# WinnerBy/PreGANPlus

Hardware: AMD Instinct MI355X
Metric: host-windows/sec (detect+diagnose+generate) (higher is better)
Workload: dtype fp32; 1 GPU; C2: PreGAN+ batched inference, 50 hosts x W=3 x 3 resources, 65536 windows per GPU, fp32; windows_per_gpu=65536, parallelism=dp1 (independent windows)

## Files before the change

preganplus_amd/csrc/pgp_decoder.hip:

```cpp
#include "pgp_device.hpp"

namespace pgp {
namespace {

constexpr int kDecWaves = 16;

template <int H>
constexpr int dec_cps() {
  int best = 1;
  for (int c = 1; c * Geo<H>::DEC_G <= 16; ++c)
    if ((H * kWindow) % c == 0) best = c;
  return best;
}

template <int H>
struct DecLds {
  static constexpr int CPS = dec_cps<H>();
  static constexpr int SLOT = CPS * Geo<H>::DEC_G * Geo<H>::FQ;
  static constexpr int TAB = Geo<H>::t_size(kMaxProtos);
  static constexpr int TOTAL = 2 * SLOT + TAB;
};

template <int H>
__global__ __launch_bounds__(kDecWaves * 64, H <= 16 ? 8 : 1) void decoder_kernel(FwdArgs a) {
  using G = Geo<H>;
  using L = DecLds<H>;
  __shared__ __attribute__((aligned(16))) float smem[L::TOTAL];
  float* tab = smem + 2 * L::SLOT;
  const int tsz = G::t_size(a.K);
  for (int i = threadIdx.x; i < tsz; i += blockDim.x) tab[i] = a.tab[i];

  const int lane = threadIdx.x & 63, g = lane >> 4, j = lane & 15;
  const int wv = __builtin_amdgcn_readfirstlane(threadIdx.x >> 6);
  const long blk = (long)blockIdx.x * kDecWaves + wv;
  const long nblk = (a.B + 15) / 16;
  const bool active = blk < nblk;
  const float* wdec = a.frags + G::OFF_DEC;
  const float* lat = a.lat + (active ? blk : 0) * G::LAT_BLK;
  constexpr int NCH = H * kWindow;

  constexpr int CPS = L::CPS, SG = CPS * G::DEC_G;
  float* cur = smem;
  float* nxt = smem + L::SLOT;
  dma_groups(wdec, cur, SG, wv, kDecWaves, lane);
  auto load_b = [&](int c, bool ok, float (&v)[G::KS_D]) {
    const float* lc = lat + (long)c * G::KS_D * 64;
#pragma unroll
    for (int q = 0; q < G::LAT_FG; ++q) {
      const f32x4 t = ok ? ld4(lc + q * 256 + lane * 4) : f32x4{0.f, 0.f, 0.f, 0.f};
#pragma unroll
      for (int e = 0; e < 4; ++e) v[4 * q + e] = t[e];
    }
#pragma unroll
    for (int r = 0; r < G::KS_D % 4; ++r) v[4 * G::LAT_FG + r] = ok ? lc[G::LAT_FG * 256 + r * 64 + lane] : 0.f;
  };
  float b[CPS][G::KS_D];
#pragma unroll
  for (int u = 0; u < CPS; ++u) load_b(u, active, b[u]);
  __syncthreads();
  if (CPS < NCH) dma_groups(wdec + (long)SG * G::FQ, nxt, SG, wv, kDecWaves, lane);

  f32x4 acc[G::MT_O];
#pragma unroll
  for (int mt = 0; mt < G::MT_O; ++mt) acc[mt] = f32x4{0.f, 0.f, 0.f, 0.f};
  constexpr int MTM = G::MT_O;

#pragma unroll 1
  for (int c0 = 0; c0 < NCH; c0 += CPS) {
    float bn[CPS][G::KS_D];
    const bool pre = active && (c0 + CPS < NCH);
#pragma unroll
    for (int u = 0; u < CPS; ++u) load_b(c0 + CPS + u, pre, bn[u]);
#pragma unroll
    for (int sub = 0; sub < CPS; ++sub) {
      const float* A = cur + sub * G::DEC_G * G::FQ;
      constexpr int AMAX = G::MT_O >= 16 ? 4 : H <= 16 ? 2 : 7;
      constexpr int NGRP = (MTM + AMAX - 1) / AMAX;
      constexpr int MH = (MTM + NGRP - 1) / NGRP;
#pragma unroll
      for (int q4 = 0; q4 < G::KQ_D; ++q4) {
#pragma unroll
        for (int m0 = 0; m0 < MTM; m0 += MH) {
          f32x4 av[MH];
#pragma unroll
          for (int i = 0; i < MH; ++i)
            if (m0 + i < MTM) av[i] = ld4(A + ((m0 + i) * G::KQ_D + q4) * 256 + lane * 4);
#pragma unroll
          for (int e = 0; e < 4; ++e)
            if (4 * q4 + e < G::KS_D)
#pragma unroll
              for (int i = 0; i < MH; ++i)
                if (m0 + i < MTM) acc[m0 + i] = mfma(av[i][e], b[sub][4 * q4 + e], acc[m0 + i]);
        }
      }
    }
#pragma unroll
    for (int u = 0; u < CPS; ++u)
#pragma unroll
      for (int s = 0; s < G::KS_D; ++s) b[u][s] = bn[u][s];
    __syncthreads();
    float* t = cur;
    cur = nxt;
    nxt = t;
    if (c0 + 2 * CPS < NCH) dma_groups(wdec + (long)(c0 + 2 * CPS) * G::DEC_G * G::FQ, nxt, SG, wv, kDecWaves, lane);
  }

  const long bw = blk * 16 + j;
  const bool valid = active && bw < a.B;
  int anyf = 0;
  const float* P = tab + G::T_PROTO;
#pragma unroll
  for (int mt = 0; mt < G::MT_O; ++mt) {
    const int host = 4 * mt + g;
    const f32x4 v = acc[mt] + ld4(tab + G::T_DEC + 16 * mt + 4 * g);
    if (host < H) {
      const float l0 = v[0], l1 = v[1];
      const float p0 = __builtin_amdgcn_rcpf(1.0f + __expf(-v[2])), p1 = __builtin_amdgcn_rcpf(1.0f + __expf(-v[3]));
      const bool an = l1 > l0;
      const float e0 = an ? p0 : 0.f, e1 = an ? p1 : 0.f;
      int cl = -1;
      if (!(e0 == 0.f && e1 == 0.f)) {
        float best = INFINITY;
        for (int k = 0; k < a.K; ++k) {
          const float d0 = e0 - P[2 * k], d1 = e1 - P[2 * k + 1];
          const float dist = (d0 * d0 + d1 * d1) * 0.5f;
          if (dist < best) {
            best = dist;
            cl = k;
          }
        }
      }
      anyf |= an ? 1 : 0;
      if (valid) {
        const long o = (bw * H + host) * 2;
        a.logits[o] = l0;
        a.logits[o + 1] = l1;
        a.protos[o] = p0;
        a.protos[o + 1] = p1;
        a.cls[bw * H + host] = cl;
        a.emb[bw * G::EP + 2 * host] = e0;
        a.emb[bw * G::EP + 2 * host + 1] = e1;
      }
    }
  }
  {
    const auto r = __builtin_amdgcn_permlane16_swap((unsigned)anyf, (unsigned)anyf, false, false);
    const int a16 = (int)(r[0] | r[1]);
    const auto q = __builtin_amdgcn_permlane32_swap((unsigned)a16, (unsigned)a16, false, false);
    anyf = (int)(q[0] | q[1]);
  }
  if (valid && g == 0) a.any_anom[bw] = anyf;
}

template <int H>
struct DecB {
  using G = Geo<H>;
  static constexpr int NB = cdiv(G::KQ_D, 2);
  static constexpr int FRC = NB * G::MT_O * 3;
  static constexpr long SIZE = (long)H * kWindow * FRC * 256;
  static constexpr int SLOT = FRC * 256;
  static constexpr int TOTAL = 2 * SLOT + G::MT_O * 16 + 2 * kMaxProtos;
};
template <int H>
constexpr bool dec_split() {
  return H >= 32 && DecB<H>::TOTAL * 4 <= 160 * 1024;
}

template <int H>
__global__ __launch_bounds__(256) void dec_split_kernel(const float* __restrict__ wdec, float* __restrict__ out) {
  using G = Geo<H>;
  using D = DecB<H>;
  const long f = (long)blockIdx.x * 4 + (threadIdx.x >> 6);
  const int lane = threadIdx.x & 63;
  if (f >= (long)H * kWindow * D::NB * G::MT_O) return;
  const int mt = (int)(f % G::MT_O);
  const long r = f / G::MT_O;
  const int blk = (int)(r % D::NB);
  const long c = r / D::NB;
  float v[8];
#pragma unroll
  for (int hq = 0; hq < 2; ++hq) {
    const int q4 = 2 * blk + hq;
    const f32x4 t = q4 < G::KQ_D ? ld4(wdec + ((c * G::DEC_G) + mt * G::KQ_D + q4) * 256 + lane * 4)
                                 : f32x4{0.f, 0.f, 0.f, 0.f};
#pragma unroll
    for (int e = 0; e < 4; ++e) v[4 * hq + e] = t[e];
  }
  u32x4 p[3];
  split8(v, p);
#pragma unroll
  for (int k = 0; k < 3; ++k) *reinterpret_cast<u32x4*>(out + (f * 3 + k) * 256 + lane * 4) = p[k];
}

#ifndef PGP_DEC_TW
#define PGP_DEC_TW 2
#endif
constexpr int kDecTW = PGP_DEC_TW;
#ifndef PGP_DEC_PF
#define PGP_DEC_PF 1
#endif
constexpr int kDecPF = PGP_DEC_PF;
#ifndef PGP_DEC_PIPE
#define PGP_DEC_PIPE 1
#endif
constexpr int kDecPipe = PGP_DEC_PIPE;

template <int H, int TW>
__global__ __launch_bounds__(kDecWaves / TW * 64, 1) void decoder_split_kernel(FwdArgs a) {
  using G = Geo<H>;
  using D = DecB<H>;
  constexpr int NWD = kDecWaves / TW;
  __shared__ __attribute__((aligned(16))) float smem[D::TOTAL];
  float* tdec = smem + 2 * D::SLOT;
  float* P = tdec + G::MT_O * 16;
  for (int i = threadIdx.x; i < G::MT_O * 16; i += blockDim.x) tdec[i] = a.tab[G::T_DEC + i];
  for (int i = threadIdx.x; i < 2 * a.K; i += blockDim.x) P[i] = a.tab[G::T_PROTO + i];

  const int lane = threadIdx.x & 63, g = lane >> 4, j = lane & 15;
  const int wv = __builtin_amdgcn_readfirstlane(threadIdx.x >> 6);
  const long blk0 = (long)blockIdx.x * kDecWaves + wv * TW;
  const long nblk = (a.B + 15) / 16;
  constexpr int NCH = H * kWindow;
  auto load_b = [&](int t, int c, bool ok, float (&v)[G::KS_D]) {
    const bool act = blk0 + t < nblk;
    const float* lc = a.lat + (act ? blk0 + t : 0) * G::LAT_BLK + (long)c * G::KS_D * 64;
    ok = ok && act;
#pragma unroll
    for (int q = 0; q < G::LAT_FG; ++q) {
      const f32x4 u = ok ? ld4(lc + q * 256 + lane * 4) : f32x4{0.f, 0.f, 0.f, 0.f};
#pragma unroll
      for (int e = 0; e < 4; ++e) v[4 * q + e] = u[e];
    }
#pragma unroll
    for (int r = 0; r < G::KS_D % 4; ++r) v[4 * G::LAT_FG + r] = ok ? lc[G::LAT_FG * 256 + r * 64 + lane] : 0.f;
  };
  float* cur = smem;
  float* nxt = smem + D::SLOT;
  dma_groups(a.decb, cur, D::FRC, wv, NWD, lane);
  float b[TW][G::KS_D], b1[TW][G::KS_D];
#pragma unroll
  for (int t = 0; t < TW; ++t) load_b(t, 0, true, b[t]);
  if constexpr (kDecPF > 1) {
#pragma unroll
    for (int t = 0; t < TW; ++t) load_b(t, 1, NCH > 1, b1[t]);
  }
  __syncthreads();
  if (NCH > 1) dma_groups(a.decb + (long)D::SLOT, nxt, D::FRC, wv, NWD, lane);

  f32x4 acc[TW][G::MT_O];
#pragma unroll
  for (int t = 0; t < TW; ++t)
#pragma unroll
    for (int mt = 0; mt < G::MT_O; ++mt) acc[t][mt] = f32x4{0.f, 0.f, 0.f, 0.f};

#pragma unroll 1
  for (int c = 0; c < NCH; ++c) {
    float bn[TW][G::KS_D];
#pragma unroll
    for (int t = 0; t < TW; ++t) load_b(t, c + kDecPF, c + kDecPF < NCH, bn[t]);
    auto planes = [&](int kb, int mt, u32x4 (&w)[3]) {
      const float* F = cur + ((kb * G::MT_O + mt) * 3) * 256 + lane * 4;
#pragma unroll
      for (int k = 0; k < 3; ++k) w[k] = *reinterpret_cast<const u32x4*>(F + k * 256);
    };
    constexpr int QN = D::NB * G::MT_O;
    constexpr int PD = kDecPipe > 0 ? kDecPipe : 1;
    u32x4 wq[PD][3];
    if constexpr (kDecPipe > 0) {
#pragma unroll
      for (int q = 0; q < PD; ++q)
        if (q < QN) planes(q / G::MT_O, q % G::MT_O, wq[q]);
    }
#pragma unroll
    for (int kb = 0; kb < D::NB; ++kb) {
      u32x4 x[TW][3];
#pragma unroll
      for (int t = 0; t < TW; ++t) {
        float v[8];
#pragma unroll
        for (int e = 0; e < 8; ++e) v[e] = 8 * kb + e < G::KS_D ? b[t][8 * kb + e] : 0.f;
        split8(v, x[t]);
      }
#pragma unroll
      for (int mt = 0; mt < G::MT_O; ++mt) {
        u32x4 w[3];
        if constexpr (kDecPipe > 0) {
          const int q = kb * G::MT_O + mt;
#pragma unroll
          for (int k = 0; k < 3; ++k) w[k] = wq[q % PD][k];
          if (q + PD < QN) planes((q + PD) / G::MT_O, (q + PD) % G::MT_O, wq[q % PD]);
          __builtin_amdgcn_sched_barrier(0);
        } else {
          planes(kb, mt, w);
        }
#pragma unroll
        for (int t = 0; t < TW; ++t) acc[t][mt] = mfma_bf6(w, x[t], acc[t][mt]);
      }
    }
#pragma unroll
    for (int t = 0; t < TW; ++t)
#pragma unroll
      for (int s = 0; s < G::KS_D; ++s) {
        if constexpr (kDecPF > 1) {
          b[t][s] = b1[t][s];
          b1[t][s] = bn[t][s];
        } else {
          b[t][s] = bn[t][s];
        }
      }
    __syncthreads();
    float* tmp = cur;
    cur = nxt;
    nxt = tmp;
    if (c + 2 < NCH) dma_groups(a.decb + (long)(c + 2) * D::SLOT, nxt, D::FRC, wv, NWD, lane);
  }

#pragma unroll
  for (int t = 0; t < TW; ++t) {
    const long blk = blk0 + t;
    const long bw = blk * 16 + j;
    const bool valid = blk < nblk && bw < a.B;
    int anyf = 0;
#pragma unroll
    for (int mt = 0; mt < G::MT_O; ++mt) {
      const int host = 4 * mt + g;
      const f32x4 v = acc[t][mt] + ld4(tdec + 16 * mt + 4 * g);
      if (host < H) {
        const float l0 = v[0], l1 = v[1];
        const float p0 = __builtin_amdgcn_rcpf(1.0f + __expf(-v[2])), p1 = __builtin_amdgcn_rcpf(1.0f + __expf(-v[3]));
        const bool an = l1 > l0;
        const float e0 = an ? p0 : 0.f, e1 = an ? p1 : 0.f;
        int cl = -1;
        if (!(e0 == 0.f && e1 == 0.f)) {
          float best = INFINITY;
          for (int k = 0; k < a.K; ++k) {
            const float d0 = e0 - P[2 * k], d1 = e1 - P[2 * k + 1];
            const float dist = (d0 * d0 + d1 * d1) * 0.5f;
            if (dist < best) {
              best = dist;
              cl = k;
            }
          }
        }
        anyf |= an ? 1 : 0;
        if (valid) {
          const long o = (bw * H + host) * 2;
          a.logits[o] = l0;
          a.logits[o + 1] = l1;
          a.protos[o] = p0;
          a.protos[o + 1] = p1;
          a.cls[bw * H + host] = cl;
          a.emb[bw * G::EP + 2 * host] = e0;
          a.emb[bw * G::EP + 2 * host + 1] = e1;
        }
      }
    }
    {
      const auto r = __builtin_amdgcn_permlane16_swap((unsigned)anyf, (unsigned)anyf, false, false);
      const int a16 = (int)(r[0] | r[1]);
      const auto q = __builtin_amdgcn_permlane32_swap((unsigned)a16, (unsigned)a16, false, false);
      anyf = (int)(q[0] | q[1]);
    }
    if (valid && g == 0) a.any_anom[bw] = anyf;
  }
}

template <int H>
hipError_t launch(const FwdArgs& a, hipStream_t st) {
  const long nblk = (a.B + 15) / 16;
  const int grid = (int)((nblk + kDecWaves - 1) / kDecWaves);
  if constexpr (dec_split<H>()) {
    if (a.decb != nullptr) {
      decoder_split_kernel<H, kDecTW><<<grid, kDecWaves / kDecTW * 64, 0, st>>>(a);
      return hipGetLastError();
    }
  }
  decoder_kernel<H><<<grid, kDecWaves * 64, 0, st>>>(a);
  return hipGetLastError();
}

template <int H>
hipError_t launch_split(const float* frags, float* decb, hipStream_t st) {
  if constexpr (dec_split<H>()) {
    const long nf = (long)H * kWindow * DecB<H>::NB * Geo<H>::MT_O;
    dec_split_kernel<H><<<(int)((nf + 3) / 4), 256, 0, st>>>(frags + Geo<H>::OFF_DEC, decb);
    return hipGetLastError();
  }
  return hipErrorInvalidValue;
}

}

hipError_t launch_decoder(const FwdArgs& a, hipStream_t st) {
  switch (a.H) {
#define CASE(h) \
  case h:       \
    return launch<h>(a, st);
    PGP_FOR_EACH_H(CASE)
#undef CASE
  }
  return hipErrorInvalidValue;
}

long decoder_split_floats(int H) {
  switch (H) {
#define CASE(h) \
  case h:       \
    return dec_split<h>() ? DecB<h>::SIZE : 0;
    PGP_FOR_EACH_H(CASE)
#undef CASE
  }
  return 0;
}

hipError_t launch_decoder_split(int H, const float* frags, float* decb, hipStream_t st) {
  switch (H) {
#define CASE(h) \
  case h:       \
    return launch_split<h>(frags, decb, st);
    PGP_FOR_EACH_H(CASE)
#undef CASE
  }
  return hipErrorInvalidValue;
}

}
```

preganplus_amd/roofline.py:

```python
from __future__ import annotations

PEAK_FP32_TFLOPS = 157.3
PEAK_HBM_GBS = 8000.0
PEAK_BF16_TFLOPS = 2500.0

W = 3
FF = 64
GAN_HIDDEN = 64


def macs_per_window(H: int) -> dict:
    d = H
    tokens = W * H
    hd = d // 2
    gat = tokens * 3 * d + 2 * tokens * d + W * H * H * d
    te = tokens * d * d
    per_token_layer = 3 * d * d + d * d + 2 * (W * hd) * 2 + 2 * FF * d
    layers = 2 * tokens * per_token_layer
    dec = (W * H * d) * (4 * H)
    gan = GAN_HIDDEN * (2 * H + H * H) + (H * H) * GAN_HIDDEN + GAN_HIDDEN * 2 * H * H + 2 * GAN_HIDDEN
    return dict(gat=gat, time_encoder=te, encoder_layers=layers, decoders=dec, gan=gan)


def flops_per_window(H: int) -> dict:
    return {k: 2 * v for k, v in macs_per_window(H).items()}


def total_flops_per_window(H: int) -> int:
    return sum(flops_per_window(H).values())


def encdec_flops_per_window(H: int) -> int:
    f = flops_per_window(H)
    return f["time_encoder"] + f["encoder_layers"] + f["decoders"]


def encoder_flops_per_window(H: int) -> int:
    f = flops_per_window(H)
    return f["time_encoder"] + f["encoder_layers"]


ENC_MFMA_PER_HOST = {16: 264, 50: 1116}


def encoder_executed_flops_per_window(H: int):
    n = ENC_MFMA_PER_HOST.get(H)
    return None if n is None else n * 2048 * H / 16


ENC_SPLIT_MFMA_PER_HOST = {50: (516, 504)}


def encoder_split(H: int) -> bool:
    return H in ENC_SPLIT_MFMA_PER_HOST


ENC_ASPLIT_MFMA_PER_HOST = {50: (48, 936)}


def encoder_split_executed_flops_per_window(H: int):
    f32, bf = ENC_ASPLIT_MFMA_PER_HOST.get(H) or ENC_SPLIT_MFMA_PER_HOST[H]
    return f32 * 2048 * H / 16, bf * 16 * 16 * 32 * 2 * H / 16


TUNE_MFMA_PER_UNIT = {
    16: {"tf_fwd_kernel": 156, "tf_bwd_ffn_kernel": 288, "tf_bwd_att_kernel": 96},
    50: {"tf_fwd_kernel": 840, "tf_bwd_ffn_kernel": 384, "tf_bwd_att_kernel": 1200},
}
TUNE_BF16_PER_UNIT = {
    16: {"tf_fwd_kernel": 0, "tf_bwd_ffn_kernel": 0, "tf_bwd_att_kernel": 0},
    50: {"tf_fwd_kernel": 288, "tf_bwd_ffn_kernel": 576, "tf_bwd_att_kernel": 144},
}
TUNE_FUSED_LAUNCHES = ("fwd layer 0", "fwd layer 1", "ffn bwd layer 1", "att bwd layer 1", "ffn bwd layer 0",
                       "att bwd layer 0")


def tf_grid(units: int, waves: int, cus: int, reserve: int = 0) -> int:
    r = max(0, min(reserve, cus // 2))
    gmax = max(1, min(cus - r, (units + waves - 1) // waves))
    m = (units + waves * gmax - 1) // (waves * gmax)
    return max(1, (units + waves * m - 1) // (waves * m))


def tune_fused_grids(H: int, B: int, B_fwd: int | None, cus: int, reserve: int = 0):
    units = (B * H + 15) // 16
    ufwd = ((B if B_fwd is None else B_fwd) * H + 15) // 16
    gf, gb = tf_grid(ufwd, 8, cus, reserve), tf_grid(units, 4, cus, reserve)
    return [gf, gf, gb, gb, gb, gb]


def tune_te_mfma(H: int) -> int:
    nt = (H + 15) // 16
    ks = 4 * (H // 16) + (min(H % 16, 4) if H % 16 else 0)
    return nt * ks * 3


def tune_fused_flops(H: int, B: int, B_fwd: int | None = None):
    c = TUNE_MFMA_PER_UNIT.get(H)
    if c is None:
        return None
    bf = TUNE_BF16_PER_UNIT.get(H, {})
    eq = {k: n * 2048 + bf.get(k, 0) * 16 * 16 * 32 * 2 * PEAK_FP32_TFLOPS / PEAK_BF16_TFLOPS for k, n in c.items()}
    units = (B * H + 15) // 16
    ufwd = ((B if B_fwd is None else B_fwd) * H + 15) // 16
    fwd, te = eq["tf_fwd_kernel"], tune_te_mfma(H) * 2048
    return ([ufwd * fwd, ufwd * (fwd - te)]
            + [units * n for n in (eq["tf_bwd_ffn_kernel"], eq["tf_bwd_att_kernel"], eq["tf_bwd_ffn_kernel"],
                                   eq["tf_bwd_att_kernel"])])


def encoder_io_bytes_per_window(H: int) -> int:
    return 4 * (W * H * 3) + 4 * (W * H * H)


def decoder_flops_per_window(H: int) -> int:
    return flops_per_window(H)["decoders"]


def decoder_split(H: int) -> bool:
    return H in (32, 50)


def gan_split(H: int) -> bool:
    return H in (16, 50)


def gan_split_flops_per_window(H: int, onehot: bool = True) -> int:
    ep = (2 * H + 15) // 16
    npe = (ep + 1) // 2
    nps = ((H * H + 15) // 16 + 1) // 2
    mtn = (H + 15) // 16
    npn = (mtn + 1) // 2
    n = npe * 4 * 6 + nps * 8 * (3 if onehot else 6) + H * (mtn * 2 * 6 + 4 * npn * 6)
    return n * 16 * 16 * 32 * 2 // 16


def decoder_split_flops_per_window(H: int) -> int:
    ks = (H + 3) // 4
    nb = ((ks + 3) // 4 + 1) // 2
    mt = (4 * H + 15) // 16
    return H * W * nb * mt * 6 * 16 * 16 * 32 * 2 // 16


def gan_flops_per_window(H: int) -> int:
    return flops_per_window(H)["gan"]


def path_bytes_per_window(H: int) -> int:
    return 36 * H + 4 * H * H + 8 * H + 8 * H + 4 * H + 4 * H + 8


def fpe_macs_per_window(H: int = 16) -> int:
    E, L = H + 3, 10
    gru = W * (9 * 3 * H + 9 * 3)
    gat = W * (H * 3 * H + 2 * H * H + H * H * H)
    mha = W * 3 * E * E + 2 * W * W * E + W * E * E
    enc = W * E * L * H
    dec = H * (2 * L + 2 * L)
    return gru + gat + mha + enc + dec


def fpe_flops_per_window(H: int = 16) -> int:
    return 2 * fpe_macs_per_window(H)


def fpe_executed_flops_per_window(H: int = 16) -> int:
    per_step = H * (27 + 6) * 2 + 27 * 2 + H * H * (2 + 4) + H * (3 + 3 + 2) * 2
    mha = 3 * (36 + 6) * 2 + 9 * 6 * 2 + 3 * 3 * 6 * 2
    out = 4 * H * 18 * 2
    return 3 * per_step + mha + out


def fpe_bytes_per_window(H: int = 16) -> int:
    return 36 * H + 12 + 8 * H + 8 * H + 4 * H + 4 + 8 * H


def tune_step_flops_per_window(H: int) -> int:
    f = flops_per_window(H)
    return 3 * (f["gat"] + f["time_encoder"] + f["encoder_layers"] + f["decoders"])


def gan_step_macs_per_env(H: int, hidden: int = GAN_HIDDEN) -> int:
    gin, hh = 2 * H + H * H, H * H
    fwd = hidden * gin + hh * hidden + hidden * 2 * hh + 2 * hidden
    disc_step = 2 * hidden + 2 * hidden + hidden * 2 * hh
    gen_step = hidden * 2 * hh + 2 * hidden + 2 * hidden + 3 * hh * hidden + hidden * gin
    return fwd + disc_step + gen_step


def gan_step_flops_per_env(H: int) -> int:
    return 2 * gan_step_macs_per_env(H)
```

Before: 694.0 million host-windows/s.

## Pack decoder K-dimension across chunk bodies to cut padded MFMA blocks

The split decoder's K reduction is repacked so several window chunks (a body of W*HB chunks) are concatenated before being cut into 8-wide MFMA blocks. Previously each chunk's K (KS_D=13 for H=50) was padded to a full 16. This removes zero-padding work and LDS weight traffic. The latent loads are rescheduled at compile time into per-block prefetch units with static_for, and each LDS slot now holds SB blocks. A waitcnt before the barrier is added to ensure the DMA has landed. The cost is more complex indexing and more register pressure from the wider b arrays.

```diff
diff --git a/preganplus_amd/csrc/pgp_decoder.hip b/preganplus_amd/csrc/pgp_decoder.hip
--- a/preganplus_amd/csrc/pgp_decoder.hip
+++ b/preganplus_amd/csrc/pgp_decoder.hip
@@ -1,3 +1,5 @@
+#include <type_traits>
+
 #include "pgp_device.hpp"
 
 namespace pgp {
@@ -152,14 +154,30 @@
   if (valid && g == 0) a.any_anom[bw] = anyf;
 }
 
+
+#ifndef PGP_DEC_HB
+#define PGP_DEC_HB 2
+#endif
+#ifndef PGP_DEC_F
+#define PGP_DEC_F 2
+#endif
 template <int H>
 struct DecB {
   using G = Geo<H>;
-  static constexpr int NB = cdiv(G::KQ_D, 2);
-  static constexpr int FRC = NB * G::MT_O * 3;
-  static constexpr long SIZE = (long)H * kWindow * FRC * 256;
-  static constexpr int SLOT = FRC * 256;
+  static constexpr int HB = G::KS_D % 8 == 0 ? 0 : H % PGP_DEC_HB == 0 ? PGP_DEC_HB : 1;
+  static constexpr int CB = HB == 0 ? 1 : kWindow * HB;
+  static constexpr int LEN = CB * G::KS_D;
+  static constexpr int BB = cdiv(LEN, 8);
+  static constexpr int F = PGP_DEC_F <= BB * 8 - LEN ? PGP_DEC_F : 0;
+  static constexpr int NBODY = H * kWindow / CB;
+  static constexpr int SB = BB % 2 == 0 ? 2 : 1;
+  static constexpr int SPB = BB / SB;
+  static constexpr int NSLOT = NBODY * SPB;
+  static constexpr int FRS = SB * G::MT_O * 3;
+  static constexpr int SLOT = FRS * 256;
+  static constexpr long SIZE = (long)NSLOT * SLOT;
   static constexpr int TOTAL = 2 * SLOT + G::MT_O * 16 + 2 * kMaxProtos;
+  static_assert(H * kWindow % CB == 0, "bodies tile the chunks");
 };
 template <int H>
 constexpr bool dec_split() {
@@ -172,19 +190,18 @@
   using D = DecB<H>;
   const long f = (long)blockIdx.x * 4 + (threadIdx.x >> 6);
   const int lane = threadIdx.x & 63;
-  if (f >= (long)H * kWindow * D::NB * G::MT_O) return;
+  if (f >= (long)D::NBODY * D::BB * G::MT_O) return;
   const int mt = (int)(f % G::MT_O);
   const long r = f / G::MT_O;
-  const int blk = (int)(r % D::NB);
-  const long c = r / D::NB;
+  const int blk = (int)(r % D::BB);
+  const long c0 = r / D::BB * D::CB;
   float v[8];
 #pragma unroll
-  for (int hq = 0; hq < 2; ++hq) {
-    const int q4 = 2 * blk + hq;
-    const f32x4 t = q4 < G::KQ_D ? ld4(wdec + ((c * G::DEC_G) + mt * G::KQ_D + q4) * 256 + lane * 4)
-                                 : f32x4{0.f, 0.f, 0.f, 0.f};
-#pragma unroll
-    for (int e = 0; e < 4; ++e) v[4 * hq + e] = t[e];
+  for (int e = 0; e < 8; ++e) {
+    const int p = 8 * blk + e - D::F;
+    const long c = c0 + p / G::KS_D;
+    const int s = p % G::KS_D;
+    v[e] = p >= 0 && p < D::LEN ? wdec[((c * G::DEC_G) + mt * G::KQ_D + s / 4) * 256 + lane * 4 + s % 4] : 0.f;
   }
   u32x4 p[3];
   split8(v, p);
@@ -196,56 +213,80 @@
 #define PGP_DEC_TW 2
 #endif
 constexpr int kDecTW = PGP_DEC_TW;
-#ifndef PGP_DEC_PF
-#define PGP_DEC_PF 1
-#endif
-constexpr int kDecPF = PGP_DEC_PF;
 #ifndef PGP_DEC_PIPE
 #define PGP_DEC_PIPE 1
 #endif
 constexpr int kDecPipe = PGP_DEC_PIPE;
+#ifndef PGP_DEC_PFD
+#define PGP_DEC_PFD 1
+#endif
+constexpr int kDecPFD = PGP_DEC_PFD;
+
+template <int I, int N, class F>
+PGP_DEV void static_for(F&& f) {
+  if constexpr (I < N) {
+    f(std::integral_constant<int, I>{});
+    static_for<I + 1, N>(f);
+  }
+}
+
+PGP_DEV void dma_landed() { __builtin_amdgcn_s_waitcnt(0x0F70); }
 
 template <int H, int TW>
 __global__ __launch_bounds__(kDecWaves / TW * 64, 1) void decoder_split_kernel(FwdArgs a) {
   using G = Geo<H>;
   using D = DecB<H>;
   constexpr int NWD = kDecWaves / TW;
+  constexpr int BB = D::BB, SB = D::SB;
+  constexpr int PFD = kDecPFD < BB ? kDecPFD : BB;
   __shared__ __attribute__((aligned(16))) float smem[D::TOTAL];
   float* tdec = smem + 2 * D::SLOT;
   float* P = tdec + G::MT_O * 16;
   for (int i = threadIdx.x; i < G::MT_O * 16; i += blockDim.x) tdec[i] = a.tab[G::T_DEC + i];
   for (int i = threadIdx.x; i < 2 * a.K; i += blockDim.x) P[i] = a.tab[G::T_PROTO + i];
 
-  const int lane = threadIdx.x & 63, g = lane >> 4, j = lane & 15;
+  const int lane = threadIdx.x & 63;
   const int wv = __builtin_amdgcn_readfirstlane(threadIdx.x >> 6);
   const long blk0 = (long)blockIdx.x * kDecWaves + wv * TW;
   const long nblk = (a.B + 15) / 16;
-  constexpr int NCH = H * kWindow;
-  auto load_b = [&](int t, int c, bool ok, float (&v)[G::KS_D]) {
-    const bool act = blk0 + t < nblk;
-    const float* lc = a.lat + (act ? blk0 + t : 0) * G::LAT_BLK + (long)c * G::KS_D * 64;
-    ok = ok && act;
-#pragma unroll
-    for (int q = 0; q < G::LAT_FG; ++q) {
-      const f32x4 u = ok ? ld4(lc + q * 256 + lane * 4) : f32x4{0.f, 0.f, 0.f, 0.f};
-#pragma unroll
-      for (int e = 0; e < 4; ++e) v[4 * q + e] = u[e];
-    }
-#pragma unroll
-    for (int r = 0; r < G::KS_D % 4; ++r) v[4 * G::LAT_FG + r] = ok ? lc[G::LAT_FG * 256 + r * 64 + lane] : 0.f;
+  auto load_units = [&](int t, int body, auto FU, float (&v)[BB * 8]) __attribute__((always_inline)) {
+    constexpr int fu = decltype(FU)::value;
+    const long tile = blk0 + t < nblk ? blk0 + t : 0;
+    const float* lb = a.lat + tile * G::LAT_BLK + (long)(body < D::NBODY ? body : 0) * D::LEN * 64;
+    static_for<0, D::CB * (G::LAT_FG + G::KS_D % 4)>([&](auto U) __attribute__((always_inline)) {
+      constexpr int ch = decltype(U)::value / (G::LAT_FG + G::KS_D % 4);
+      constexpr int q = decltype(U)::value % (G::LAT_FG + G::KS_D % 4);
+      constexpr int p0 = D::F + ch * G::KS_D + (q < G::LAT_FG ? 4 * q : 3 * G::LAT_FG + q);
+      if constexpr (p0 / 8 == fu) {
+        unsigned off = (unsigned)lane * (q < G::LAT_FG ? 16u : 4u);
+        asm volatile("" : "+v"(off));
+        const float* lc = reinterpret_cast<const float*>(reinterpret_cast<const char*>(lb + ch * G::KS_D * 64) + off);
+        if constexpr (q < G::LAT_FG) {
+          const f32x4 u = ld4(lc + q * 256);
+          v[p0] = u[0];
+          v[p0 + 1] = u[1];
+          v[p0 + 2] = u[2];
+          v[p0 + 3] = u[3];
+        } else {
+          v[p0] = lc[G::LAT_FG * 256 + (q - G::LAT_FG) * 64];
+        }
+      }
+    });
   };
   float* cur = smem;
   float* nxt = smem + D::SLOT;
-  dma_groups(a.decb, cur, D::FRC, wv, NWD, lane);
-  float b[TW][G::KS_D], b1[TW][G::KS_D];
-#pragma unroll
-  for (int t = 0; t < TW; ++t) load_b(t, 0, true, b[t]);
-  if constexpr (kDecPF > 1) {
-#pragma unroll
-    for (int t = 0; t < TW; ++t) load_b(t, 1, NCH > 1, b1[t]);
-  }
+  dma_groups(a.decb, cur, D::FRS, wv, NWD, lane);
+  float b[TW][BB * 8];
+#pragma unroll
+  for (int t = 0; t < TW; ++t) {
+#pragma unroll
+    for (int p = 0; p < BB * 8; ++p)
+      if (p < D::F || p >= D::F + D::LEN) b[t][p] = 0.f;
+    static_for<0, PFD>([&](auto FU) __attribute__((always_inline)) { load_units(t, 0, FU, b[t]); });
+  }
+  dma_landed();
   __syncthreads();
-  if (NCH > 1) dma_groups(a.decb + (long)D::SLOT, nxt, D::FRC, wv, NWD, lane);
+  if (D::NSLOT > 1) dma_groups(a.decb + (long)D::SLOT, nxt, D::FRS, wv, NWD, lane);
 
   f32x4 acc[TW][G::MT_O];
 #pragma unroll
@@ -254,67 +295,69 @@
     for (int mt = 0; mt < G::MT_O; ++mt) acc[t][mt] = f32x4{0.f, 0.f, 0.f, 0.f};
 
 #pragma unroll 1
-  for (int c = 0; c < NCH; ++c) {
-    float bn[TW][G::KS_D];
-#pragma unroll
-    for (int t = 0; t < TW; ++t) load_b(t, c + kDecPF, c + kDecPF < NCH, bn[t]);
-    auto planes = [&](int kb, int mt, u32x4 (&w)[3]) {
-      const float* F = cur + ((kb * G::MT_O + mt) * 3) * 256 + lane * 4;
-#pragma unroll
-      for (int k = 0; k < 3; ++k) w[k] = *reinterpret_cast<const u32x4*>(F + k * 256);
-    };
-    constexpr int QN = D::NB * G::MT_O;
-    constexpr int PD = kDecPipe > 0 ? kDecPipe : 1;
-    u32x4 wq[PD][3];
-    if constexpr (kDecPipe > 0) {
-#pragma unroll
-      for (int q = 0; q < PD; ++q)
-        if (q < QN) planes(q / G::MT_O, q % G::MT_O, wq[q]);
-    }
-#pragma unroll
-    for (int kb = 0; kb < D::NB; ++kb) {
-      u32x4 x[TW][3];
-#pragma unroll
-      for (int t = 0; t < TW; ++t) {
-        float v[8];
-#pragma unroll
-        for (int e = 0; e < 8; ++e) v[e] = 8 * kb + e < G::KS_D ? b[t][8 * kb + e] : 0.f;
-        split8(v, x[t]);
-      }
-#pragma unroll
-      for (int mt = 0; mt < G::MT_O; ++mt) {
-        u32x4 w[3];
-        if constexpr (kDecPipe > 0) {
-          const int q = kb * G::MT_O + mt;
-#pragma unroll
-          for (int k = 0; k < 3; ++k) w[k] = wq[q % PD][k];
-          if (q + PD < QN) planes((q + PD) / G::MT_O, (q + PD) % G::MT_O, wq[q % PD]);
-          __builtin_amdgcn_sched_barrier(0);
-        } else {
-          planes(kb, mt, w);
-        }
-#pragma unroll
-        for (int t = 0; t < TW; ++t) acc[t][mt] = mfma_bf6(w, x[t], acc[t][mt]);
-      }
-    }
-#pragma unroll
-    for (int t = 0; t < TW; ++t)
-#pragma unroll
-      for (int s = 0; s < G::KS_D; ++s) {
-        if constexpr (kDecPF > 1) {
-          b[t][s] = b1[t][s];
-          b1[t][s] = bn[t][s];
-        } else {
-          b[t][s] = bn[t][s];
-        }
-      }
-    __syncthreads();
-    float* tmp = cur;
-    cur = nxt;
-    nxt = tmp;
-    if (c + 2 < NCH) dma_groups(a.decb + (long)(c + 2) * D::SLOT, nxt, D::FRC, wv, NWD, lane);
-  }
-
+  for (int body = 0; body < D::NBODY; ++body) {
+    static_for<0, D::SPB>([&](auto S) __attribute__((always_inline)) {
+      constexpr int s = decltype(S)::value;
+      auto planes = [&](int kb, int mt, u32x4 (&w)[3]) {
+        const float* F = cur + ((kb * G::MT_O + mt) * 3) * 256 + lane * 4;
+#pragma unroll
+        for (int k = 0; k < 3; ++k) w[k] = *reinterpret_cast<const u32x4*>(F + k * 256);
+      };
+      constexpr int QN = SB * G::MT_O;
+      constexpr int PD = kDecPipe > 0 ? kDecPipe : 1;
+      u32x4 wq[PD][3];
+      if constexpr (kDecPipe > 0) {
+#pragma unroll
+        for (int q = 0; q < PD; ++q)
+          if (q < QN) planes(q / G::MT_O, q % G::MT_O, wq[q]);
+      }
+      static_for<0, SB>([&](auto KB) __attribute__((always_inline)) {
+        constexpr int kb = decltype(KB)::value;
+        constexpr int blk = s * SB + kb;
+        u32x4 x[TW][3];
+#pragma unroll
+        for (int t = 0; t < TW; ++t) {
+          float v[8];
+#pragma unroll
+          for (int e = 0; e < 8; ++e) v[e] = b[t][8 * blk + e];
+          split8(v, x[t]);
+        }
+        __builtin_amdgcn_sched_barrier(0);
+#pragma unroll
+        for (int t = 0; t < TW; ++t) {
+          if constexpr (blk + PFD < BB)
+            load_units(t, body, std::integral_constant<int, blk + PFD>{}, b[t]);
+          else
+            load_units(t, body + 1, std::integral_constant<int, blk + PFD - BB>{}, b[t]);
+        }
+#pragma unroll
+        for (int mt = 0; mt < G::MT_O; ++mt) {
+          u32x4 w[3];
+          if constexpr (kDecPipe > 0) {
+            const int q = kb * G::MT_O + mt;
+#pragma unroll
+            for (int k = 0; k < 3; ++k) w[k] = wq[q % PD][k];
+            if (q + PD < QN) planes((q + PD) / G::MT_O, (q + PD) % G::MT_O, wq[q % PD]);
+            __builtin_amdgcn_sched_barrier(0);
+          } else {
+            planes(kb, mt, w);
+          }
+#pragma unroll
+          for (int t = 0; t < TW; ++t) acc[t][mt] = mfma_bf6(w, x[t], acc[t][mt]);
+        }
+      });
+      dma_landed();
+      __syncthreads();
+      float* tmp = cur;
+      cur = nxt;
+      nxt = tmp;
+      const int sg = body * D::SPB + s;
+      if (sg + 2 < D::NSLOT) dma_groups(a.decb + (long)(sg + 2) * D::SLOT, nxt, D::FRS, wv, NWD, lane);
+    });
+  }
+
+  const int el = __builtin_amdgcn_mbcnt_hi(~0u, __builtin_amdgcn_mbcnt_lo(~0u, 0u));
+  const int g = el >> 4, j = el & 15;
 #pragma unroll
   for (int t = 0; t < TW; ++t) {
     const long blk = blk0 + t;
@@ -382,7 +425,7 @@
 template <int H>
 hipError_t launch_split(const float* frags, float* decb, hipStream_t st) {
   if constexpr (dec_split<H>()) {
-    const long nf = (long)H * kWindow * DecB<H>::NB * Geo<H>::MT_O;
+    const long nf = (long)DecB<H>::NBODY * DecB<H>::BB * Geo<H>::MT_O;
     dec_split_kernel<H><<<(int)((nf + 3) / 4), 256, 0, st>>>(frags + Geo<H>::OFF_DEC, decb);
     return hipGetLastError();
   }
diff --git a/preganplus_amd/roofline.py b/preganplus_amd/roofline.py
--- a/preganplus_amd/roofline.py
+++ b/preganplus_amd/roofline.py
@@ -137,9 +137,10 @@
 
 def decoder_split_flops_per_window(H: int) -> int:
     ks = (H + 3) // 4
-    nb = ((ks + 3) // 4 + 1) // 2
+    cb = 1 if ks % 8 == 0 else W * (2 if H % 2 == 0 else 1)
+    blocks = H * W // cb * ((cb * ks + 7) // 8)
     mt = (4 * H + 15) // 16
-    return H * W * nb * mt * 6 * 16 * 16 * 32 * 2 // 16
+    return blocks * mt * 6 * 16 * 16 * 32 * 2 // 16
 
 
 def gan_flops_per_window(H: int) -> int:
```

Measured after the change: 719.2 million host-windows/s, median of 6. 1.04x the previous value.
